# niclasborlin/dbat

Measured on AMD Instinct MI355X. Metric: LM iterations/sec, higher is better.
Workload: dtype f64

## Files before the change

### dbat_amd/csrc/dbat_core.hip

```cpp
#include <hip/hip_runtime.h>
#include <rocblas/rocblas.h>
#include <rocsolver/rocsolver.h>
#include <rccl/rccl.h>

#include <chrono>
#include <cmath>
#include <cstdio>
#include <cstdlib>
#include <memory>
#include <string>
#include <thread>
#include <type_traits>
#include <utility>
#include <atomic>
#include <vector>

#include "../../include/dbat_hip.h"
#include "chol_df.hpp"
#include "kernels.hpp"
#include "sig.hpp"
#include "heavy.hpp"
#include "plan.hpp"
#include "resect.hpp"
#include "robust.hpp"
// ... 492 lines not shown
            if (allreduce(allreduce_user, buf, count, (void *)stream) != 0) throw DeviceError{"all-reduce callback failed"};
        }
    }
    const double *gathered(const double *z_dev) {
        if (!multi()) return z_dev;
        if (!zgather.p) zgather.alloc((size_t)P.NZ);
        launch<k_mask_owned>(dim3((unsigned)cdiv(P.NZ, 256)), dim3(256), 0, P.NZ, z_mine.p, z_dev, zgather.p);
        do_allreduce(zgather.p, P.NZ);
        return zgather.p;
    }
    void read_scal(double *host, int n) {
        if (n <= 32) {
            HIPCHK(hipMemcpyAsync(hpin, scal.p, n * sizeof(double), hipMemcpyDeviceToHost, stream));
            sync();
            memcpy(host, hpin, n * sizeof(double));
            return;
        }
        HIPCHK(hipMemcpyAsync(host, scal.p, n * sizeof(double), hipMemcpyDeviceToHost, stream));
        sync();
    }
    void prep_cams(const double *zz, CamRec *into = nullptr) {
        if (!into) { into = cams.p; cams_at_lin = false; }
        launch<k_cam_prep>(dim3((unsigned)cdiv(P.nc, 64)), dim3(64), 0, d, zz, into);
    }
    void x_to_z(const double *x_host, double *z_dev) {
        HIPCHK(hipMemcpyAsync(z_dev, P.z0.data(), P.NZ * 8, hipMemcpyHostToDevice, stream));
        if (P.n) {
            HIPCHK(hipMemcpyAsync(xbuf.p, x_host, P.n * 8, hipMemcpyHostToDevice, stream));
            launch<k_scatter_x>(dim3((unsigned)cdiv(P.n, 256)), dim3(256), 0, P.n, x2z.p, xbuf.p, z_dev);
        }
    }
    void z_to_x(const double *z_dev, double *x_host) {
        if (!P.n) return;
        stage(4);
        z_dev = gathered(z_dev);
        launch<k_gather_x>(dim3((unsigned)cdiv(P.n, 256)), dim3(256), 0, P.n, x2z.p, z_dev, xbuf.p);
        HIPCHK(hipMemcpyAsync(x_host, xbuf.p, P.n * 8, hipMemcpyDeviceToHost, stream));
        sync();
    }

    DevBuf<double> trace_dev;
    int trace_cap = 0, trace_n = 0;
    std::vector<uint8_t> trace_have;
    void trace_begin() { trace_n = 0; trace_have.clear(); }
    void trace_put(int k, const double *z_dev) {
        if (!P.n || k < 0) return;
        if (k >= trace_cap) {
            const int cap = std::max(8, std::max(2 * trace_cap, k + 1));
            DevBuf<double> nb;
            nb.alloc((size_t)P.n * cap);
            if (trace_cap > 0) HIPCHK(hipMemcpyAsync(nb.p, trace_dev.p, (size_t)P.n * trace_cap * 8, hipMemcpyDeviceToDevice, stream));
            HIPCHK(hipStreamSynchronize(stream));
            std::swap(trace_dev.p, nb.p);
            trace_cap = cap;
        }
        stage(4);
        z_dev = gathered(z_dev);
        launch<k_gather_x>(dim3((unsigned)cdiv(P.n, 256)), dim3(256), 0, P.n, x2z.p, z_dev, trace_dev.p + (size_t)P.n * k);
        if ((int)trace_have.size() <= k) trace_have.resize((size_t)k + 1, 0);
        trace_have[k] = 1;
        trace_n = std::max(trace_n, k + 1);
    }
    void trace_truncate(int n) { trace_n = std::min(trace_n, std::max(n, 0)); }
    int trace_download(double *host, int cap_cols) {
        const int nt = std::min(trace_n, cap_cols);
        if (!P.n || nt <= 0) return std::max(nt, 0);
        HIPCHK(hipMemcpyAsync(host, trace_dev.p, (size_t)P.n * nt * 8, hipMemcpyDeviceToHost, stream));
        HIPCHK(hipStreamSynchronize(stream));
        for (int k = 0; k < nt; ++k)
            if (!trace_have[k]) std::fill(host + (size_t)P.n * k, host + (size_t)P.n * (k + 1), NAN);
        if ((size_t)P.n * trace_cap * 8 > ((size_t)256 << 20)) {
            DevBuf<double> old;
            std::swap(old.p, trace_dev.p);
            trace_cap = 0;
        }
        return nt;
    }

    double eval_f_step(const double *x, double alpha, const double *pdir, double *out) {
        stage(3);
        if ((int64_t)cdiv(P.NZ, 256) < P.nc) { axpby(1.0, x, alpha, pdir, out); return eval_f(out, nullptr, nullptr); }
        launch<k_axpby_cams>(dim3((unsigned)cdiv(P.NZ, 256)), dim3(256), 0, d, 1.0, x, alpha, pdir, out, cams_f.p);
        return eval_f(out, nullptr, nullptr, true);
    }
    double eval_f(const double *zz, double *r_w_out, double *r_unw_out, bool cams_ready = false) {
        stage(3);
        if (!cams_ready) prep_cams(zz, cams_f.p);
        mark(6);
        const bool res_tail = n_cm_chunks_all > 0 && n_cm_chunks_all <= 512 && !d.any_prior && !multi() && !r_w_out && !r_unw_out;
        with_value<2, 3, 4, 5>(P.model, [&](auto M) {
            with_value<false, true>(uv_pre, [&](auto PRE) {
                if (n_cm_chunks_all > 0)
                    launch<k_residual_cm<M, PRE>>(dim3((unsigned)n_cm_chunks_all), dim3(256), 0, d, zz, cams_f.p, cm_pt.p, cm_uv.p, pw ? cm_w.p : (const double *)nullptr,
                                                  cm_chunk_cam.p, cm_chunk_start.p, partial.p, res_tail ? gctr.p + 1 : (unsigned *)nullptr, scal.p, hpin, res_tail ? ++mb_seq : 0ull);
                mark(7);
                if (r_w_out || r_unw_out) launch<k_residual<M, PRE>>(dim3(grid_obs), dim3(256), 0, d, zz, cams_f.p, rpart.p, r_w_out, r_unw_out);
            });
        });
        if (!res_tail)
            launch<k_prior_sq>(dim3(grid_zs), dim3(1024), 0, d, zz, gpart.p, gctr.p + 1, (const double *)partial.p, n_cm_chunks_all,
                               scal.p, multi() ? (double *)nullptr : hpin, ++mb_seq);
        double s;
        if (multi()) { do_allreduce(scal.p, 1); read_scal(&s, 1); }
        else { mb_armed = true; sync(); s = hpin[0]; }
        ++n_res_evals;
        return 0.5 * s;
    }

    int det_ncx() const { return P.ncolmax <= 6 ? 6 : (P.ncolmax <= 14 ? 14 : 15); }
    bool deterministic_supported() const { return P.nranks == 1 && !P.shared_eo && P.ncolmax <= 15 && n_cm_chunks_all > 0; }
    void set_deterministic(bool on) {
        if (on && !deterministic_supported())
            throw UsageError{"deterministic mode: one rank, no shared EO blocks (camera stations), at most nine estimated IO columns per camera"};
        if (on && !det_u.p) {
            const int nc = P.nc;
            det_cam_part.alloc((size_t)std::max<int64_t>(n_cm_chunks_all, 1) * DET_CP);
            det_io_part.alloc((size_t)nc * DET_IOP);
            det_rr.alloc((size_t)nc + 1 + DET_PRIOR_PARTS);
            det_u.alloc((size_t)P.NS + 1);
            std::vector<int32_t> cr((size_t)2 * (2 * nc + 1), 0);
            for (int part = 0; part < 2; ++part) {
                const int64_t q0 = part == 0 ? 0 : n_cm_chunks, q1 = part == 0 ? n_cm_chunks : n_cm_chunks_all;
                int32_t *r = cr.data() + part * (2 * nc + 1);
                for (int c = 0; c < nc; ++c) { r[2 * c] = (int32_t)q1; r[2 * c + 1] = (int32_t)q1; }
                for (int64_t q = q0; q < q1; ++q) {
                    const int c = P.cm_chunk_cam[q];
                    if (r[2 * c] == (int32_t)q1) r[2 * c] = (int32_t)q;
                    r[2 * c + 1] = (int32_t)q + 1;
                }
                for (int c = 0; c < nc; ++c) if (r[2 * c] == (int32_t)q1) r[2 * c + 1] = (int32_t)q1;
            }
            det_cam_chunks.upload(cr);
        }
        deterministic = on;
        d.deterministic = on ? 1 : 0;
        d.det_cam_part = det_cam_part.p; d.det_io_part = det_io_part.p; d.det_rr = det_rr.p; d.det_u = det_u.p;
        d.det_cam_chunks = det_cam_chunks.p;
    }
    const double *det_z = nullptr;
    void det_camera_side() {
        const int nio = (int)P.nIOu;
        const int ncx = det_ncx();
        with_value<6, 14, 15>(ncx, [&](auto NCX) { launch<k_det_cam_reduce<NCX>>(dim3((unsigned)P.nc), dim3(256), 0, d, cams.p, S, g_c, g_red, diagU); });
        if (ncx > 6 && nio > 0) launch<k_det_io_reduce<15>>(dim3((unsigned)(nio * (nio + 1) / 2 + nio)), dim3(256), 0, d, cams.p, nio, S, g_c, g_red, diagU);
        if (d.any_prior) launch<k_det_prior_sq>(dim3(DET_PRIOR_PARTS), dim3(256), 0, d, det_z);
        launch<k_det_rows>(dim3((unsigned)cdiv(P.NS, 256)), dim3(256), 0, d, (const double *)diagU);
        if (ncx == 6) launch<k_det_round_cam<6>>(dim3((unsigned)P.nc), dim3(256), 0, d, cams.p, 0, S, g_red);
        else launch<k_det_round_cam<15>>(dim3((unsigned)P.nc + 1), dim3(256), 0, d, cams.p, nio, S, g_red);
    }

    void cam_normal(const double *zz, int64_t q0, int64_t nq, int ncx) {
        const double *w = pw ? cm_w.p : (const double *)nullptr;
        with_value<2, 3, 4, 5>(P.model, [&](auto M) { with_value<6, 14, 15>(ncx, [&](auto NCX) {
            if constexpr (NCX == 6)
                launch<k_cam_normal6<M>>(dim3((unsigned)nq), dim3(256), 0, d, zz, cams.p, cm_pt.p, cm_uv.p, w, cm_chunk_cam.p + q0, cm_chunk_start.p + q0, S, g_c, g_red, diagU);
            else
                launch<k_cam_normal<M, NCX>>(dim3((unsigned)nq), dim3(256), 0, d, zz, cams.p, cm_pt.p, cm_uv.p, w, cm_chunk_cam.p + q0, cm_chunk_start.p + q0, S, g_c, g_red, diagU);
        }); });
    }

    void build_enqueue(const double *zz, double lambda, int scale) {
        stage(0);
        const bool fused_first = !s_dense_dirty && P.NS >= P.nc;
        if (!fused_first) prep_cams(zz);
        else cams_at_lin = false;
        bool pivmm_set = false;
        if (s_dense_dirty) {
            HIPCHK(hipMemsetAsync(red.p, 0, red_count * sizeof(double), stream));
            s_dense_dirty = false;
        } else {
            launch<k_envelope_cams>(dim3((unsigned)P.NS), dim3(256), 0, d, zz, cams.p, S, ldS, (int)P.NS, env_tail0, col_bend.p, g_red, pivmm.p);
            pivmm_set = true;
        }
        if (!pivmm_set) HIPCHK(hipMemcpyAsync(pivmm.p, hpin + 48, 4 * sizeof(double), hipMemcpyHostToDevice, stream));
        int64_t npart = 0;
        const bool det_list = deterministic && route != TileRoute::sig;
        const int64_t nb_tiled = det_list ? 0 : P.nb_tiled;
        if (deterministic) {
            cam_normal(zz, 0, n_cm_chunks_all, det_ncx());
            det_z = zz;
            det_camera_side();
        }
        if (ntiles > 0 && nb_tiled > 0) {
            npart = ntiles;
            if (!deterministic && use_tile2 && tile_ncx <= 15 && n_cm_chunks > 0) cam_normal(zz, 0, n_cm_chunks, tile_ncx);
            mark(0);
            with_value<2, 3, 4, 5>(P.model, [&](auto M) {
                if (route == TileRoute::sig) {
                    with_value<6, 14>(tile_ncx, [&](auto NCX) { with_value<4, 5>(sig_rb, [&](auto RB) { with_value<false, true>(pw, [&](auto PW) {
                        launch<k_build_sig<M, RB, NCX, PW>>(dim3((unsigned)std::min<int64_t>(ntiles, n_cu)), dim3(64 * sig_waves(RB, NCX > 6)), sig_lds_bytes(RB, NCX > 6),
                                                            d, zz, cams.p, lambda, scale, S, g_red, Vinv.p, gp.p, jn2p.p, partial.p, pivmm.p, sg_chunk.p, sg_tile_chunk0.p,
                                                            sg_lc.p, sg_uv.p, PW ? sg_w.p : (const double *)nullptr, gctr.p + 5);
                    }); }); });
                } else if (route == TileRoute::tile3) {
                    launch<k_build_tile3<M, TILE3_PC, TILE3_NBUF>>(dim3((unsigned)ntiles), dim3(768), lds_tile3, d, zz, cams.p, lambda, scale, S, g_red, Vinv.p, gp.p,
                                                                   jn2p.p, partial.p, pivmm.p);
                } else {
                    with_value<14, 15>(tile_ncx, [&](auto NCX) {
                        launch<k_build_tile2<M, NCX, TILE2_PC, TILE2_NBUF>>(dim3((unsigned)ntiles), dim3(512), lds_tile2, d, zz, cams.p, lambda, scale, S, g_c, g_red,
                                                                            diagU, Vinv.p, gp.p, jn2p.p, partial.p, pivmm.p);
                    });
                }
            });
            mark(1);
        }
        const bool no_tiles = !(ntiles > 0 && nb_tiled > 0);
        if (no_tiles) mark(0);
        const int64_t nb_lists = use_heavy ? P.nb_tiled : nb;
        if (nb_lists > nb_tiled) {
            with_value<2, 3, 4, 5>(P.model, [&](auto M) { with_value<false, true>(P.with_io, [&](auto IO) {
                launch<k_build<M, IO>>(dim3((unsigned)(nb_lists - nb_tiled)), dim3(P.BT), lds_build, d, zz, cams.p, lambda, scale, S, g_c, g_red, diagU, Vinv.p, gp.p,
                                       jn2p.p, partial.p + npart, pivmm.p, (int)nb_tiled);
            }); });
            npart += nb_lists - nb_tiled;
        }
        if (use_heavy) {
            mark(10);
            if (!deterministic && n_cm_chunks_all > n_cm_chunks) cam_normal(zz, n_cm_chunks, n_cm_chunks_all - n_cm_chunks, tile_ncx);
            if (nb > P.nb_tiled) {
                with_value<2, 3, 4, 5>(P.model, [&](auto M) { with_value<6, 14, 15>(tile_ncx, [&](auto NCX) {
                    launch<k_heavy_z<M, NCX>>(dim3((unsigned)(nb - P.nb_tiled)), dim3(256), heavy_z_lds_bytes(NCX, P.hv_max_batch_slots, deterministic), d, hv, zz,
                                              cams.p, lambda, scale, hv_Z.p, Vinv.p, gp.p, jn2p.p, partial.p + npart, pivmm.p, (int)P.nb_tiled);
                }); });
                npart += nb - P.nb_tiled;
            }
            if (ngiant > 0) {
                with_value<2, 3, 4, 5>(P.model, [&](auto M) { with_value<6, 14, 15>(tile_ncx, [&](auto NCX) {
                    launch<k_heavy_z_giant<M, NCX>>(dim3((unsigned)ngiant), dim3(giant_threads), 0, d, hv, zz, cams.p, lambda, scale, hv_Z.p, Vinv.p, gp.p, jn2p.p,
                                                    partial.p + npart, pivmm.p);
                }); });
                npart += ngiant;
            }
            mark(11);
            launch<k_heavy_syrk>(dim3((unsigned)cdiv(hv.ntasks, 4)), dim3(256), 0, d, hv, (const double *)hv_Z.p, S, g_red);
            mark(12);
        }
        if (no_tiles) mark(1);
        if (ngiant > 0 && !use_heavy) {
            with_value<2, 3, 4, 5>(P.model, [&](auto M) { with_value<false, true>(P.with_io, [&](auto IO) {
                launch<k_build_giant<M, IO>>(dim3((unsigned)ngiant), dim3(giant_threads), 0, d, zz, cams.p, lambda, scale, S, g_c, g_red, diagU, Vinv.p, gp.p, jn2p.p,
                                             partial.p + npart, pivmm.p);
            }); });
            npart += ngiant;
        }
        if (deterministic && route == TileRoute::sig && !no_tiles) {
            HIPCHK(hipMemcpyAsync(hpin + 60, gctr.p + 7, sizeof(unsigned), hipMemcpyDeviceToHost, stream));
            det_timeout_pending = true;
        }
        if ((d.ablate & 32) && use_heavy && nb > P.nb_tiled) {
            unsigned long long h[16];
            HIPCHK(hipStreamSynchronize(stream));
            HIPCHK(hipMemcpyFromSymbol(h, HIP_SYMBOL(g_tile2_prof), sizeof(h)));
            static const char *nm[6] = {"evaluate", "V, g sums", "point blocks", "EO rows of Z", "IO rows of Z", "tail"};
            fprintf(stderr, "[heavy_z prof, us per batch (thread 0) avg over %d batches]", (int)(nb - P.nb_tiled));
            for (int i = 0; i < 6; ++i) fprintf(stderr, " %s=%.2f", nm[i], h[8 + i] * 0.01 / (double)std::max<int64_t>(nb - P.nb_tiled, 1));
            fprintf(stderr, "\n");
            for (int i = 8; i < 16; ++i) h[i] = 0;
            HIPCHK(hipMemcpyToSymbol(HIP_SYMBOL(g_tile2_prof), h, sizeof(h)));
        }
        if ((d.ablate & 32) && use_sig) {
            unsigned long long h[16];
            HIPCHK(hipStreamSynchronize(stream));
            HIPCHK(hipMemcpyFromSymbol(h, HIP_SYMBOL(g_tile2_prof), sizeof(h)));
            static const char *nm[8] = {"tile init", "chunk head", "pass 1", "pass 2 eval+write", "pass 2 mfma", "chunk flush", "wait for the tile", "tile flush"};
            fprintf(stderr, "[sig prof, us per tile (wave 0) avg over %d tiles]", (int)ntiles);
            for (int i = 0; i < 8; ++i) fprintf(stderr, " %s=%.2f", nm[i], h[i] * 0.01 / (double)std::max<int64_t>(ntiles, 1));
            fprintf(stderr, "\n");
            memset(h, 0, sizeof(h));
            HIPCHK(hipMemcpyToSymbol(HIP_SYMBOL(g_tile2_prof), h, sizeof(h)));
        } else if ((d.ablate & 32) && use_tile2) {
            unsigned long long h[16];
            HIPCHK(hipStreamSynchronize(stream));
            HIPCHK(hipMemcpyFromSymbol(h, HIP_SYMBOL(g_tile2_prof), sizeof(h)));
            static const char *nm[12] = {"stage(wait freed)", "P1", "pbarrier", "P2", "P3", "drain", "cons wait full", "cons zero+free", "tail/flush", "loop head", "cons product", "cons wait done"};
            fprintf(stderr, "[tile2 prof, us per tile avg over %d tiles]", (int)ntiles);
            for (int i = 0; i < 12; ++i) fprintf(stderr, " %s=%.2f", nm[i], h[i] * 0.01 / (double)std::max<int64_t>(ntiles, 1));
            fprintf(stderr, "\n");
            memset(h, 0, sizeof(h));
            HIPCHK(hipMemcpyToSymbol(HIP_SYMBOL(g_tile2_prof), h, sizeof(h)));
        }
        launch<k_build_tail>(dim3(grid_zs), dim3(1024), 0, d, zz, partial.p, npart, jn2p.p, gpart.p, gctr.p + 2, red_scal,
                zz != zlin.p ? zlin.p : (double *)nullptr);
    }
    bool pend_build = false;
    double pend_lambda = 0;
    int pend_scale = 0;
    void request_build(double lambda, int scale) {
        pend_build = true; pend_lambda = lambda; pend_scale = scale;
        lambda_lin = lambda; scale_lin = scale;
    }
    void ensure_build() {
        if (!pend_build) return;
        build(z.p, pend_lambda, pend_scale, true);
    }
    void settle_lin_point() {
        if (!pend_build) return;
        copy(zlin.p, z.p);
        cams_at_lin = false; s_valid = false; have_lin = true;
    }
    void allreduce_vectors() {
        if (!multi()) return;
        do_allreduce(g_c, 2 * P.NS + 8);
    }
    void trace_only_pass(const double *zz) {
        stage(0);
        prep_cams(zz);
        if (n_cm_chunks_all > 0) {
            with_value<2, 3, 4, 5>(P.model, [&](auto M) { with_value<6, 14, 15, MAXCOL>(tile_ncx, [&](auto NCX) {
                launch<k_trace_cm<M, NCX>>(dim3((unsigned)n_cm_chunks_all), dim3(256), 0, d, zz, cams.p, cm_pt.p, cm_uv.p, pw ? cm_w.p : (const double *)nullptr,
// ... 2376 lines not shown
```

### dbat_amd/csrc/kernels.hpp

```cpp
#pragma once
#include <hip/hip_runtime.h>

#include "model.hpp"

namespace dbat {

struct DevProblem {
    int nc, np, nIOrows, nK, nP, nIOu, ncolmax, BT;
    int64_t NS, NZ, nobs, nb;
    int64_t ldS;
    const int32_t *cam_ncol, *cam_col, *cam_iorow;
    const uint32_t *cam_eo_est;
    const int32_t *io_src;
    const double *io_fixed;
    const double *px;
    const double *cam_w;
    const uint8_t *z_est, *z_mine;
    const double *z_prw, *z_prv;
    const int32_t *o_cam, *o_pt;
    const double *o_uv;
    const double *o_uv_raw;
    int uv_pre;
    const double *o_w;
    const uint32_t *o_seg;
// ... 968 lines not shown
    const int k = (int)(o1 - o0);
    const int pt = d.o_pt[o0];
    double s[3] = {0, 0, 0};
    for (int i = t; i < k; i += BT) {
        const int64_t o = o0 + i;
        const CamRec &C = cams[d.o_cam[o]];
        const int ncol = WITH_IO ? C.ncol : 6;
        double r[2], E[2][NCX], B[2][3], tt[2] = {0, 0};
        eval_obs_cols<MODEL, WITH_IO>(d, C, z, o, pt, r, E, B);
#pragma unroll
        for (int a = 0; a < NCX; ++a)
            if (a < ncol) { const double dc = dz[C.col[a]]; tt[0] += E[0][a] * dc; tt[1] += E[1][a] * dc; }
        s[0] = fma2(s[0], B[0][0], tt[0], B[1][0], tt[1]);
        s[1] = fma2(s[1], B[0][1], tt[0], B[1][1], tt[1]);
        s[2] = fma2(s[2], B[0][2], tt[0], B[1][2], tt[1]);
    }
    block_sum<3>(s, sh);
    if (t == 0) {
        for (int q = 0; q < 3; ++q) s[q] += gp[3 * (int64_t)pt + q];
        double p0, p1, p2;
        point_block_solve_neg(Vinv + 6 * (int64_t)pt, s[0], s[1], s[2], p0, p1, p2);
        const int64_t zp = d.NS + 3 * (int64_t)pt;
        dps[0] = d.z_est[zp] ? p0 : 0.0; dps[1] = d.z_est[zp + 1] ? p1 : 0.0; dps[2] = d.z_est[zp + 2] ? p2 : 0.0;
        dz[zp] = dps[0]; dz[zp + 1] = dps[1]; dz[zp + 2] = dps[2];
    }
    __syncthreads();
    double acc[2] = {0, 0};
    for (int i = t; i < k; i += BT) {
        const int64_t o = o0 + i;
        const CamRec &C = cams[d.o_cam[o]];
        const int ncol = WITH_IO ? C.ncol : 6;
        double r[2], E[2][NCX], B[2][3], tt[2] = {0, 0};
        eval_obs_cols<MODEL, WITH_IO>(d, C, z, o, pt, r, E, B);
#pragma unroll
        for (int a = 0; a < NCX; ++a)
            if (a < ncol) { const double dc = dz[C.col[a]]; tt[0] += E[0][a] * dc; tt[1] += E[1][a] * dc; }
        const double j0 = tt[0] + B[0][0] * dps[0] + B[0][1] * dps[1] + B[0][2] * dps[2];
        const double j1 = tt[1] + B[1][0] * dps[0] + B[1][1] * dps[1] + B[1][2] * dps[2];
        acc[0] = fma2(acc[0], j0, j0, j1, j1);
    }
    block_sum<2>(acc, sh);
    if (t == 0) { partial[2 * blockIdx.x] = acc[0]; partial[2 * blockIdx.x + 1] = acc[1]; }
}

typedef double mfma_d4 __attribute__((ext_vector_type(4)));
constexpr int TILE_LD = 144;

__device__ __forceinline__ void lds_fence() {
    __builtin_amdgcn_s_waitcnt(0xc07f);
    asm volatile("" ::: "memory");
}

template <int MODEL, int NCX>
__global__ __launch_bounds__(256, 3) void k_cam_normal(DevProblem d, const double *__restrict__ z,
                                                       const CamRec *__restrict__ cams,
                                                       const int32_t *__restrict__ cm_pt, const double *__restrict__ cm_uv,
                                                       const double *__restrict__ cm_w,
                                                       const int32_t *__restrict__ chunk_cam,
                                                       const int64_t *__restrict__ chunk_start, double *__restrict__ S,
                                                       double *__restrict__ g_c, double *__restrict__ g_red,
                                                       double *__restrict__ diagU) {
    constexpr bool IO = NCX > 6;
    constexpr int GLD = 66;
    __shared__ double Gl[4 * 16 * GLD];
    const int t = threadIdx.x, lane = t & 63, w = t >> 6;
    const int cam = chunk_cam[blockIdx.x];
    const int64_t q0 = chunk_start[blockIdx.x], q1 = chunk_start[blockIdx.x + 1];
    const CamRec &C = cams[cam];
    const int ncol = IO ? min(C.ncol, NCX) : 6;
    double *Gw = Gl + w * 16 * GLD;
    for (int c = NCX + 1; c < 16; ++c) Gw[c * GLD + lane] = 0.0;
    mfma_d4 acc = {0, 0, 0, 0};
    {
        auto load_obs = [&](int64_t q, int &pt, double2 &uv, double2 &ww) {
            pt = 0; uv = double2{0, 0}; ww = double2{C.w[0], C.w[1]};
            if (q < q1) {
                pt = cm_pt[q];
                uv = reinterpret_cast<const double2 *>(cm_uv)[q];
                if (cm_w) ww = reinterpret_cast<const double2 *>(cm_w)[q];
            }
        };
        const int64_t qw = q0 + 64 * w + lane;
        int pt_a, pt_b;
        double2 uv_a, uv_b, w_a, w_b;
        load_obs(qw, pt_a, uv_a, w_a);
        load_obs(qw + 256, pt_b, uv_b, w_b);
        double Qn[3];
        { const int64_t zp = d.NS + 3 * (int64_t)pt_a; Qn[0] = z[zp]; Qn[1] = z[zp + 1]; Qn[2] = z[zp + 2]; }
        const int prow = lane & 31;
        const double *ga = Gw + (lane & 15) * GLD + (lane >> 4);
        for (int64_t base = q0 + 64 * w; base < q1; base += 256) {
            const int64_t q = base + lane;
            const double Q[3] = {Qn[0], Qn[1], Qn[2]};
            const double2 uv = uv_a, ww = w_a;
            pt_a = pt_b; uv_a = uv_b; w_a = w_b;
            { const int64_t zp = d.NS + 3 * (int64_t)pt_a; Qn[0] = z[zp]; Qn[1] = z[zp + 1]; Qn[2] = z[zp + 2]; }
            load_obs(q + 512, pt_b, uv_b, w_b);
            double r[2] = {0, 0}, E[2][NCX];
#pragma unroll
            for (int c = 0; c < NCX; ++c) { E[0][c] = 0.0; E[1][c] = 0.0; }
            if (q < q1) {
                double B[2][3];
                eval_obs_pre<MODEL, NCX>(d, C, Q, uv.x, uv.y, ww.x, ww.y, 7u, r, E, B);
            }
#pragma unroll
            for (int half = 0; half < 2; ++half) {
                if ((lane >> 5) == half) {
                    if (ncol == NCX) {
#pragma unroll
                        for (int c = 0; c < NCX; ++c) { Gw[c * GLD + prow] = E[0][c]; Gw[c * GLD + 32 + prow] = E[1][c]; }
                    } else {
#pragma unroll
                        for (int c = 0; c < NCX; ++c) {
                            const bool on = c < ncol;
                            Gw[c * GLD + prow] = on ? E[0][c] : 0.0;
                            Gw[c * GLD + 32 + prow] = on ? E[1][c] : 0.0;
                        }
                    }
                    Gw[NCX * GLD + prow] = r[0]; Gw[NCX * GLD + 32 + prow] = r[1];
                }
                lds_fence();
                if (base + 32 * half < q1) {
                    double av[16];
#pragma unroll
                    for (int kk = 0; kk < 16; ++kk) av[kk] = ga[4 * kk];
#pragma unroll
                    for (int kk = 0; kk < 16; ++kk) acc = __builtin_amdgcn_mfma_f64_16x16x4f64(av[kk], av[kk], acc, 0, 0, 0);
                }
                lds_fence();
            }
        }
    }
    double *Gs = Gl;
    __syncthreads();
#pragma unroll
    for (int e = 0; e < 4; ++e) Gs[w * 256 + ((lane >> 4) + 4 * e) * 16 + (lane & 15)] = acc[e];
    __syncthreads();
    const int i = t >> 4, j = t & 15;
    const double g = (Gs[t] + Gs[256 + t]) + (Gs[512 + t] + Gs[768 + t]);
    if (d.deterministic) { d.det_cam_part[(int64_t)blockIdx.x * DET_CP + t] = g; return; }
    if (i < ncol && g != 0.0) {
        const int64_t ri = C.col[i];
        if (j < ncol) {
            const int64_t rj = C.col[j];
            if (i > j) atomic_add_f64(S + (ri >= rj ? rj * d.ldS + ri : ri * d.ldS + rj), g);
            else if (i == j) { atomic_add_f64(S + ri * d.ldS + ri, g); atomic_add_f64(diagU + ri, g); }
        } else if (j == NCX) {
            atomic_add_f64(g_c + ri, g);
            atomic_add_f64(g_red + ri, g);
        }
    }
}

template <int MODEL>
__global__ __launch_bounds__(256) void k_cam_normal6(DevProblem d, const double *__restrict__ z,
                                                     const CamRec *__restrict__ cams,
                                                     const int32_t *__restrict__ cm_pt, const double *__restrict__ cm_uv,
                                                     const double *__restrict__ cm_w,
                                                     const int32_t *__restrict__ chunk_cam,
                                                     const int64_t *__restrict__ chunk_start, double *__restrict__ S,
                                                     double *__restrict__ g_c, double *__restrict__ g_red,
                                                     double *__restrict__ diagU) {
    __shared__ double Gs[4 * 28];
    __shared__ double Rd[4][14 * 65];
    const int t = threadIdx.x, lane = t & 63, w = t >> 6;
    const int cam = chunk_cam[blockIdx.x];
    const int64_t q0 = chunk_start[blockIdx.x], q1 = chunk_start[blockIdx.x + 1];
    const CamRec &C = cams[cam];
    double G[28];
#pragma unroll
    for (int i = 0; i < 28; ++i) G[i] = 0.0;
    const double2 *uvp = reinterpret_cast<const double2 *>(cm_uv), *wp = reinterpret_cast<const double2 *>(cm_w);
    for (int64_t qb = q0 + t; qb < q1; qb += 4 * 256) {
        int pt[4]; double2 uv[4], ww[4]; double Qv[4][3];
#pragma unroll
        for (int u = 0; u < 4; ++u) {
            const int64_t q = qb + 256 * u;
            const bool on = q < q1;
            pt[u] = on ? cm_pt[q] : -1;
            uv[u] = on ? uvp[q] : double2{0, 0};
            ww[u] = (on && cm_w) ? wp[q] : double2{C.w[0], C.w[1]};
        }
#pragma unroll
        for (int u = 0; u < 4; ++u) {
            const double *p = z + d.NS + 3 * (int64_t)(pt[u] < 0 ? 0 : pt[u]);
            Qv[u][0] = p[0]; Qv[u][1] = p[1]; Qv[u][2] = p[2];
        }
#pragma unroll
        for (int u = 0; u < 4; ++u) {
            if (pt[u] < 0) continue;
            const double d0 = Qv[u][0] - C.c[0], d1 = Qv[u][1] - C.c[1], d2 = Qv[u][2] - C.c[2];
            const double X0 = C.Mt[0] * d0 + C.Mt[1] * d1 + C.Mt[2] * d2;
            const double X1 = C.Mt[3] * d0 + C.Mt[4] * d1 + C.Mt[5] * d2;
            const double X2 = C.Mt[6] * d0 + C.Mt[7] * d1 + C.Mt[8] * d2;
            const double iz = recip(X2);
            const double ph0 = X0 * iz, ph1 = X1 * iz;
            const double nf = -C.f, sc = nf * iz, s0 = sc * ww[u].x, s1 = sc * ww[u].y;
            const double r0 = (nf * ph0 - uv[u].x) * ww[u].x, r1 = (nf * ph1 - uv[u].y) * ww[u].y;
            double y[3][3];
            angle_terms(C, d0, d1, d2, X0, X1, X2, y);
            double e0[6], e1[6];
#pragma unroll
            for (int k = 0; k < 3; ++k) {
                e0[k] = -s0 * (C.Mt[k] - ph0 * C.Mt[6 + k]);      e1[k] = -s1 * (C.Mt[3 + k] - ph1 * C.Mt[6 + k]);
                e0[3 + k] = s0 * (y[k][0] - ph0 * y[k][2]);       e1[3 + k] = s1 * (y[k][1] - ph1 * y[k][2]);
            }
            int n = 0;
#pragma unroll
            for (int i = 0; i < 6; ++i)
#pragma unroll
                for (int j = 0; j <= i; ++j, ++n) G[n] = __builtin_fma(e0[i], e0[j], __builtin_fma(e1[i], e1[j], G[n]));
#pragma unroll
            for (int i = 0; i < 6; ++i) G[21 + i] = __builtin_fma(e0[i], r0, __builtin_fma(e1[i], r1, G[21 + i]));
            G[27] = __builtin_fma(r0, r0, __builtin_fma(r1, r1, G[27]));
        }
    }
#pragma unroll
    for (int h = 0; h < 2; ++h) {
#pragma unroll
        for (int v = 0; v < 14; ++v)
            Rd[w][v * 65 + lane] = G[14 * h + v];
        lds_fence();
        __builtin_amdgcn_wave_barrier();
        const int v = lane & 15, q4 = lane >> 4;
        double sum = 0.0;
        if (v < 14) {
#pragma unroll
            for (int i = 0; i < 16; ++i) sum += Rd[w][v * 65 + 16 * q4 + i];
        }
        sum += __shfl_xor(sum, 16, 64);
        sum += __shfl_xor(sum, 32, 64);
        if (lane < 14) Gs[w * 28 + 14 * h + lane] = sum;
        lds_fence();
        __builtin_amdgcn_wave_barrier();
    }
    __syncthreads();
    if (d.deterministic) {
        if (t < 28) d.det_cam_part[(int64_t)blockIdx.x * DET_CP + t] = (Gs[t] + Gs[28 + t]) + (Gs[56 + t] + Gs[84 + t]);
        return;
    }
    if (t < 27) {
        double g = (Gs[t] + Gs[28 + t]) + (Gs[56 + t] + Gs[84 + t]);
        int i = t - 21, j = i;
        if (t < 21) {
            i = 0;
            while ((i + 1) * (i + 2) / 2 <= t) ++i;
            j = t - i * (i + 1) / 2;
        }
        if (!((C.eo_est >> i) & (C.eo_est >> j) & 1u)) g = 0.0;
        if (g != 0.0) {
            if (t < 21) {
                const int64_t ri = C.col[i], rj = C.col[j];
                if (i == j) { atomic_add_f64(S + ri * d.ldS + ri, g); atomic_add_f64(diagU + ri, g); }
                else atomic_add_f64(S + (ri >= rj ? rj * d.ldS + ri : ri * d.ldS + rj), g);
            } else {
                const int64_t ri = C.col[t - 21];
                atomic_add_f64(g_c + ri, g);
                atomic_add_f64(g_red + ri, g);
            }
        }
    }
}

template <int NCX>
__global__ __launch_bounds__(256) void k_det_cam_reduce(DevProblem d, const CamRec *__restrict__ cams, double *__restrict__ S,
                                                        double *__restrict__ g_c, double *__restrict__ g_red,
                                                        double *__restrict__ diagU) {
    const int cam = blockIdx.x, t = threadIdx.x;
    const CamRec &C = cams[cam];
    const int nel = NCX == 6 ? 28 : 256;
    double g = 0.0;
    if (t < nel) {
        for (int part = 0; part < 2; ++part) {
            const int q0 = d.det_cam_chunks[2 * cam + part * (2 * d.nc + 1)], q1 = d.det_cam_chunks[2 * cam + 1 + part * (2 * d.nc + 1)];
            for (int q = q0; q < q1; ++q) g += d.det_cam_part[(int64_t)q * DET_CP + t];
        }
    }
    if constexpr (NCX == 6) {
        if (t == 27) d.det_rr[cam] = g;
        if (t < 27) {
            int i = t - 21, j = i;
            if (t < 21) {
                i = 0;
                while ((i + 1) * (i + 2) / 2 <= t) ++i;
                j = t - i * (i + 1) / 2;
            }
            if (!((C.eo_est >> i) & (C.eo_est >> j) & 1u)) g = 0.0;
            if (t < 21) {
                const int64_t ri = C.col[i], rj = C.col[j];
                if (((C.eo_est >> i) & (C.eo_est >> j) & 1u)) {
                    S[(ri >= rj ? rj * d.ldS + ri : ri * d.ldS + rj)] = g;
                    if (i == j) diagU[ri] = g;
                }
            } else if ((C.eo_est >> i) & 1u) {
                const int64_t ri = C.col[i];
                g_c[ri] = g; g_red[ri] = g;
            }
        }
    } else {
        const int ncol = min(C.ncol, NCX);
        const int i = t >> 4, j = t & 15;
        if (i == NCX && j == NCX) d.det_rr[cam] = g;
        double *iop = d.det_io_part + (int64_t)cam * DET_IOP;
        if (i < ncol) {
            const int64_t ri = C.col[i];
            if (j < ncol && i >= j) {
                if (j >= 6) iop[(i - 6) * 9 + (j - 6)] = g;
                else {
                    const int64_t rj = C.col[j];
                    S[(ri >= rj ? rj * d.ldS + ri : ri * d.ldS + rj)] = g;
                    if (i == j) diagU[ri] = g;
                }
            } else if (j == NCX) {
                if (i >= 6) iop[81 + (i - 6)] = g;
                else { g_c[ri] = g; g_red[ri] = g; }
            }
        }
    }
}

template <int NCX>
__global__ __launch_bounds__(256) void k_det_io_reduce(DevProblem d, const CamRec *__restrict__ cams, int nio, double *__restrict__ S,
                                                       double *__restrict__ g_c, double *__restrict__ g_red,
                                                       double *__restrict__ diagU) {
    __shared__ double sh[256];
    const int npair = nio * (nio + 1) / 2, e = blockIdx.x, t = threadIdx.x;
    int p, q;
    if (e < npair) { p = 0; while ((p + 1) * (p + 2) / 2 <= e) ++p; q = e - p * (p + 1) / 2; }
    else { p = e - npair; q = -1; }
    const int64_t rp = 6 * (int64_t)d.nc + p, rq = 6 * (int64_t)d.nc + q;
    double s = 0.0;
    for (int c = t; c < d.nc; c += 256) {
        const CamRec &C = cams[c];
        const int ncol = min(C.ncol, NCX);
        int a = -1, b = -1;
        for (int k = 6; k < ncol; ++k) { if (C.col[k] == rp) a = k; if (C.col[k] == rq) b = k; }
        if (a < 0) continue;
        const double *iop = d.det_io_part + (int64_t)c * DET_IOP;
        if (q < 0) s += iop[81 + (a - 6)];
        else if (b >= 0) s += iop[(max(a, b) - 6) * 9 + (min(a, b) - 6)];
    }
    sh[t] = s;
    __syncthreads();
    for (int w = 128; w > 0; w >>= 1) {
        if (t < w) sh[t] += sh[t + w];
        __syncthreads();
    }
    if (t == 0) {
        if (q < 0) { g_c[rp] = sh[0]; g_red[rp] = sh[0]; }
        else { S[rq * d.ldS + rp] = sh[0]; if (p == q) diagU[rp] = sh[0]; }
    }
}

constexpr int DET_PRIOR_PARTS = 256;
__global__ __launch_bounds__(256) void k_det_prior_sq(DevProblem d, const double *__restrict__ z) {
    __shared__ double sh[256];
    const int t = threadIdx.x;
    const int64_t per = (d.NZ + DET_PRIOR_PARTS - 1) / DET_PRIOR_PARTS;
    const int64_t lo = per * blockIdx.x, hi = lo + per < d.NZ ? lo + per : d.NZ;
    double s = 0.0;
    for (int64_t i = lo + t; i < hi; i += 256) {
        const double pw = d.z_prw[i];
        if (pw > 0) { const double e = z[i] - d.z_prv[i]; s += pw * e * e; }
    }
    sh[t] = s;
    __syncthreads();
    for (int w = 128; w > 0; w >>= 1) {
        if (t < w) sh[t] += sh[t + w];
// ... 1510 lines not shown
```

### dbat_amd/csrc/sig.hpp

```cpp
#pragma once
#include <cstddef>
#include <type_traits>

#include "kernels.hpp"

namespace dbat {

constexpr int SIG_LDK = 18;
constexpr int SIG_PPR = 6;
constexpr int SIG_KMAXR = 13;
constexpr int SIG_NW = 8;
constexpr int SIG_CAMW = (int)(offsetof(CamRec, ncol) / 8) + 1;
constexpr int SIG_CAMW_IO = (int)((sizeof(CamRec) + 7) / 8);
constexpr int SIG_STILE = 8064;
#ifndef DBAT_SIG_IO_WAVES
#define DBAT_SIG_IO_WAVES 4
#endif
constexpr int SIG_IO_CAMS = DBAT_SIG_IO_WAVES == 8 ? 16 : 21;
__host__ __device__ constexpr int sig_stile(bool io) { return io && DBAT_SIG_IO_WAVES == 8 ? 6336 : SIG_STILE; }
__host__ __device__ constexpr int sig_cams(bool io) { return io ? SIG_IO_CAMS : 21; }

struct SigLds {
    int next_chunk, abort_;
    int flush_turn;
// ... 526 lines not shown
                if (ks + 1 < 5) load_ops(ks + 1, nxt);
                if (ks < ksteps) {
#pragma unroll
                    for (int r1 = 0; r1 < RB; ++r1)
                        if (r1 < rbk) {
#pragma unroll
                            for (int r2 = 0; r2 <= r1; ++r2)
                                acc[r1 * (r1 + 1) / 2 + r2] = __builtin_amdgcn_mfma_f64_16x16x4f64(
                                    cur[r1], cur[r2], acc[r1 * (r1 + 1) / 2 + r2], 0, 0, 0);
                        }
                }
            }
            lds_fence();
            __builtin_amdgcn_wave_barrier();
            lap(4);
        }
        if (d.deterministic) {
            volatile int *turn = &sy.flush_turn;
            int spins = 0;
            for (; *turn != ch_cur - ch0 && spins < (1 << 24); ++spins) __builtin_amdgcn_s_sleep(1);
            if (spins >= (1 << 24) && lane == 0) atomicAdd(det_timeouts, 1u);
        }
        {
            const int r6k = ry;
            int tcm[RB];
#pragma unroll
            for (int r2 = 0; r2 < RB; ++r2) tcm[r2] = sy.tmap[wave][min(16 * r2 + (lane & 15), 79)];
#pragma unroll
            for (int r1 = 0; r1 < RB; ++r1) {
                if (r1 >= rbk) break;
#pragma unroll
                for (int e = 0; e < 4; ++e) {
                    const int lr = 16 * r1 + (lane >> 4) + 4 * e;
                    const bool yrow = lr == r6k;
                    double *row = stile + (yrow ? STILE : sy.toff[wave][min(lr, 79)]);
                    if (!DBAT_ABLATE(d, 8)) {
#pragma unroll
                        for (int r2 = 0; r2 < r1; ++r2) {
                            const double v = acc[r1 * (r1 + 1) / 2 + r2][e];
                            atomic_add_f64(row + tcm[r2], yrow ? -v : v);
                        }
                        const double v = acc[r1 * (r1 + 1) / 2 + r1][e];
                        const int lcol = 16 * r1 + (lane & 15);
                        if (lcol <= lr && lcol < r6k && v != 0.0) atomic_add_f64(row + tcm[r1], yrow ? -v : v);
                    }
                }
            }
        }
        if (d.deterministic) {
            lds_fence();
            if (lane == 0) { volatile int *turn = &sy.flush_turn; *turn = ch_cur - ch0 + 1; }
        }
        __builtin_amdgcn_wave_barrier();
        lap(5);
    }
    lap(6);
    __syncthreads();
    lap(6);
    {
        constexpr int NCOLW = (128 + NW - 1) / NW;
        double v0[NCOLW], v1[NCOLW];
#pragma unroll
        for (int q = 0; q < NCOLW; ++q) {
            const int tc = wave + q * NW, tr = tc + lane;
            v0[q] = (tc < nrows && tr < nrows) ? stile[tr * (tr + 1) / 2 + tc] : 0.0;
            v1[q] = (tc < nrows && tr + 64 < nrows) ? stile[(tr + 64) * (tr + 65) / 2 + tc] : 0.0;
            if (d.deterministic && tc < nrows) {
                const double uc = sy.urow[tc];
                if (tr < nrows) v0[q] = det_round(v0[q], sy.urow[tr], uc);
                if (tr + 64 < nrows) v1[q] = det_round(v1[q], sy.urow[tr + 64], uc);
            }
        }
        if (!DBAT_ABLATE(d, 16)) {
#pragma unroll
            for (int q = 0; q < NCOLW; ++q) {
                const int tc = wave + q * NW, tr = tc + lane;
                if (tc < nrows) {
                    const int64_t gcol = sy.grow[tc] * d.ldS;
                    if (v0[q] != 0.0) atomic_add_f64(S + gcol + sy.grow[tr], -v0[q]);
                    if (v1[q] != 0.0) atomic_add_f64(S + gcol + sy.grow[tr + 64], -v1[q]);
                }
            }
        }
    }
    for (int i = t; i < nrows; i += NT) {
        const double v = d.deterministic ? det_round(vt[i], sy.urow[i], sy.uf) : vt[i];
        if (v != 0.0) atomic_add_f64(g_red + sy.grow[i], v);
    }
    double accr[1] = {rr};
    block_sum<1>(accr, sh);
    if (t == 0) partial[part_slot] = accr[0];
    pmin = pmin < 1e300 ? sqrt(pmin) : pmin; pmax = sqrt(pmax);
    for (int off = 32; off > 0; off >>= 1) {
        pmin = fmin(pmin, __shfl_down(pmin, off, 64));
        pmax = fmax(pmax, __shfl_down(pmax, off, 64));
    }
    if ((t & 63) == 0 && pmax > 0.0) {
        atomicMin(pivmm, (unsigned long long)__double_as_longlong(pmin));
        atomicMax(pivmm + 1, (unsigned long long)__double_as_longlong(pmax));
    }
    lap(7);
    if (prof)
        for (int i = 0; i < 8; ++i) if (tp[i]) atomicAdd(&g_tile2_prof[i], (unsigned long long)tp[i]);
}

template <int MODEL, int RB, int NCX, bool PW>
__global__ __launch_bounds__(64 * sig_waves(RB, (NCX > 6))) void k_build_sig(DevProblem d, const double *__restrict__ z,
                                                   const CamRec *__restrict__ cams, double lambda, int scale,
                                                   double *__restrict__ S, double *__restrict__ g_red,
                                                   double *__restrict__ Vinv, double *__restrict__ gp,
                                                   double *__restrict__ jn2p,
                                                   double *__restrict__ partial, unsigned long long *__restrict__ pivmm,
                                                   const int32_t *__restrict__ sg_chunk,
                                                   const int32_t *__restrict__ sg_tile_chunk0,
                                                   const uint8_t *__restrict__ sg_lc, const double *__restrict__ sg_uv,
                                                   const double *__restrict__ sg_w, unsigned *__restrict__ tile_ctr) {
    __shared__ unsigned s_ticket;
    __shared__ SigLds sy;
    __shared__ double sh[16];
    for (;;) {
        if (threadIdx.x == 0) s_ticket = __hip_atomic_fetch_add(tile_ctr, 1u, __ATOMIC_RELAXED, __HIP_MEMORY_SCOPE_AGENT);
        __syncthreads();
        const unsigned ti = s_ticket;
        if (ti >= (unsigned)d.ntiles) {
            if (threadIdx.x == 0 && ti == (unsigned)d.ntiles + gridDim.x - 1)
                __hip_atomic_store(tile_ctr, 0u, __ATOMIC_RELAXED, __HIP_MEMORY_SCOPE_AGENT);
            return;
        }
        const int tile = d.tile_order[ti];
        int ios = 0;
        if constexpr (NCX > 6) ios = d.tile_io_simple ? d.tile_io_simple[tile] : 0;
#ifdef DBAT_SIG_ONLY_IOS
        ios = DBAT_SIG_ONLY_IOS;
#endif
        if (NCX > 6 && ios == 1)
            build_sig_tile<MODEL, RB, NCX, (NCX > 6 ? 1 : 0), PW>(d, tile, (int)ti, z, cams, lambda, scale, S, g_red, Vinv, gp, jn2p, partial, pivmm, sg_chunk, sg_tile_chunk0, sg_lc, sg_uv, sg_w, tile_ctr + 2, sy, sh);
        else if (NCX > 6 && ios == 2)
            build_sig_tile<MODEL, RB, NCX, (NCX > 6 ? 2 : 0), PW>(d, tile, (int)ti, z, cams, lambda, scale, S, g_red, Vinv, gp, jn2p, partial, pivmm, sg_chunk, sg_tile_chunk0, sg_lc, sg_uv, sg_w, tile_ctr + 2, sy, sh);
        else
            build_sig_tile<MODEL, RB, NCX, 0, PW>(d, tile, (int)ti, z, cams, lambda, scale, S, g_red, Vinv, gp, jn2p, partial, pivmm, sg_chunk, sg_tile_chunk0, sg_lc, sg_uv, sg_w, tile_ctr + 2, sy, sh);
        __syncthreads();
    }
}

template <int MODEL, int NCX>
__global__ __launch_bounds__(256) void k_backsub_sig(DevProblem d, const double *__restrict__ z,
                                                     const CamRec *__restrict__ cams,
                                                     const double *__restrict__ Vinv, const double *__restrict__ gp,
                                                     double *__restrict__ dz, double *__restrict__ partial ,
                                                     const int32_t *__restrict__ sg_chunk, int nchunks,
                                                     const int32_t *__restrict__ sg_gcam,
                                                     const double *__restrict__ sg_uv, const double *__restrict__ sg_w) {
    constexpr int CW = (int)((sizeof(CamRec) + 7) / 8);
    __shared__ double sh[8];
    __shared__ double crec[4][SIG_KMAXR][CW];
    __shared__ double dcs[4][SIG_KMAXR][NCX];
    const int t = threadIdx.x, lane = t & 63;
    const int wv = t >> 6;
    const int ch = __builtin_amdgcn_readfirstlane(blockIdx.x * 4 + (t >> 6));
    double acc[2] = {0, 0};
    if (ch < nchunks) {
        const int32_t *cd = sg_chunk + 8 * (int64_t)ch;
        const int pt0 = cd[0], npts = cd[1], k = cd[2], gm = cd[4], gi0 = cd[5], uv0 = cd[6];
        const int mycam = lane < k ? sg_gcam[16 * (int64_t)ch + lane] : 0;
        for (int base = 0; base < k * CW; base += 64) {
            const int idx = base + lane, c = min(idx / CW, k - 1), f = idx - c * CW;
            const int cam = __builtin_amdgcn_ds_bpermute(4 * c, mycam);
            if (idx < k * CW) crec[wv][c][f] = reinterpret_cast<const double *>(cams + cam)[f];
        }
        __builtin_amdgcn_wave_barrier();
        for (int idx = lane; idx < k * NCX; idx += 64) {
            const int c = idx / NCX, a = idx - c * NCX;
            const CamRec &C = *reinterpret_cast<const CamRec *>(crec[wv][c]);
            const bool on = a < (NCX > 6 ? min(C.ncol, NCX) : 6) && (NCX > 6 || ((C.eo_est >> a) & 1u));
            dcs[wv][c][a] = on ? dz[C.col[a]] : 0.0;
        }
        __builtin_amdgcn_wave_barrier();
        const int G = npts > 32 ? 64 : (npts > 16 ? 32 : (npts > 8 ? 16 : 8));
        const int pi = lane & (G - 1), jh = lane / G, jstep = 64 / G;
        const bool act = pi < npts;
        const int pt = pt0 + (act ? pi : 0);
        const int64_t zp = d.NS + 3 * (int64_t)pt;
        const double Q[3] = {z[zp], z[zp + 1], z[zp + 2]};
        const unsigned est = (d.z_est[zp] ? 1u : 0u) | (d.z_est[zp + 1] ? 2u : 0u) | (d.z_est[zp + 2] ? 4u : 0u);
        const double2 *uvp = reinterpret_cast<const double2 *>(sg_uv), *wp = reinterpret_cast<const double2 *>(sg_w);
        const int64_t q0 = uv0 + gi0 + (act ? pi : 0);
        double sB[3] = {0, 0, 0}, V0[6] = {0, 0, 0, 0, 0, 0}, tt2 = 0;
        auto sweep = [&](auto per_obs_w) {
        for (int j = jh; j < k; j += jstep) {
            const CamRec &C = *reinterpret_cast<const CamRec *>(crec[wv][j]);
            double2 uv = {0, 0};
            if constexpr (NCX > 6) uv = uvp[q0 + (int64_t)j * gm];
            double w0, w1;
            if constexpr (decltype(per_obs_w)::value) { const double2 ww = wp[q0 + (int64_t)j * gm]; w0 = ww.x; w1 = ww.y; }
            else { w0 = C.w[0]; w1 = C.w[1]; }
            double B[2][3], t0 = 0, t1 = 0;
            if constexpr (NCX > 6) {
                obs_step_dot<MODEL, true>(C, Q, uv.x, uv.y, w0, w1, est, dcs[wv][j], t0, t1, B);
            } else {
                sig_step_dot6(C, Q, w0, w1, dcs[wv][j], t0, t1, B);
            }
#define DBAT_ACC2(acc, a, b, c, e) acc = __builtin_fma(a, b, __builtin_fma(c, e, acc))
            DBAT_ACC2(tt2, t0, t0, t1, t1);
            DBAT_ACC2(sB[0], B[0][0], t0, B[1][0], t1);
            DBAT_ACC2(sB[1], B[0][1], t0, B[1][1], t1);
            DBAT_ACC2(sB[2], B[0][2], t0, B[1][2], t1);
            DBAT_ACC2(V0[0], B[0][0], B[0][0], B[1][0], B[1][0]);
            DBAT_ACC2(V0[1], B[0][0], B[0][1], B[1][0], B[1][1]);
            DBAT_ACC2(V0[2], B[0][0], B[0][2], B[1][0], B[1][2]);
            DBAT_ACC2(V0[3], B[0][1], B[0][1], B[1][1], B[1][1]);
            DBAT_ACC2(V0[4], B[0][1], B[0][2], B[1][1], B[1][2]);
            DBAT_ACC2(V0[5], B[0][2], B[0][2], B[1][2], B[1][2]);
#undef DBAT_ACC2
        }
        };
        if (sg_w) sweep(std::true_type{}); else sweep(std::false_type{});
        for (int m = G; m < 64; m <<= 1) {
#pragma unroll
            for (int c = 0; c < 3; ++c) sB[c] += lane_get(sB[c], lane ^ m);
#pragma unroll
            for (int c = 0; c < 6; ++c) V0[c] += lane_get(V0[c], lane ^ m);
            tt2 += lane_get(tt2, lane ^ m);
        }
        {
            const double s0 = gp[3 * (int64_t)pt] + sB[0], s1 = gp[3 * (int64_t)pt + 1] + sB[1], s2 = gp[3 * (int64_t)pt + 2] + sB[2];
            double p0, p1, p2;
            point_block_solve_neg(Vinv + 6 * (int64_t)pt, s0, s1, s2, p0, p1, p2);
            const double d0 = (est & 1u) ? p0 : 0.0, d1 = (est & 2u) ? p1 : 0.0, d2 = (est & 4u) ? p2 : 0.0;
            if (act && lane == pi) {
                dz[zp] = d0; dz[zp + 1] = d1; dz[zp + 2] = d2;
                acc[0] = tt2 + 2.0 * (d0 * sB[0] + d1 * sB[1] + d2 * sB[2])
                       + d0 * (V0[0] * d0 + V0[1] * d1 + V0[2] * d2) + d1 * (V0[1] * d0 + V0[3] * d1 + V0[4] * d2)
                       + d2 * (V0[2] * d0 + V0[4] * d1 + V0[5] * d2);
            }
        }
    }
    block_sum<2>(acc, sh);
    if (t == 0) { partial[2 * blockIdx.x] = acc[0]; partial[2 * blockIdx.x + 1] = acc[1]; }
}

}
```

Before: 631.9.

## Software-pipeline camera-normal loads and prefetch camera records in signature backsub

The 6-column camera normal kernel now runs a fixed three-stage software pipeline (index/uv loads, point gathers, math) over four batches of two observations. The per-observation weight path is specialised at compile time, and a static_assert ties the chunk size to this schedule. The signature back-substitution kernel reads its chunk descriptor and camera ids through one lane-parallel load plus readlane. It stages only the needed CamRec fields and camera deltas in registers before writing them to LDS, and issues the point gradient and Vinv loads early so their latency overlaps. The aim is to hide global-memory latency, at the cost of more registers and less generality (fixed chunk size, hardcoded CamRec field offsets).

```diff
diff --git a/dbat_amd/csrc/dbat_core.hip b/dbat_amd/csrc/dbat_core.hip
--- a/dbat_amd/csrc/dbat_core.hip
+++ b/dbat_amd/csrc/dbat_core.hip
@@ -668,9 +668,12 @@
     void cam_normal(const double *zz, int64_t q0, int64_t nq, int ncx) {
         const double *w = pw ? cm_w.p : (const double *)nullptr;
         with_value<2, 3, 4, 5>(P.model, [&](auto M) { with_value<6, 14, 15>(ncx, [&](auto NCX) {
-            if constexpr (NCX == 6)
-                launch<k_cam_normal6<M>>(dim3((unsigned)nq), dim3(256), 0, d, zz, cams.p, cm_pt.p, cm_uv.p, w, cm_chunk_cam.p + q0, cm_chunk_start.p + q0, S, g_c, g_red, diagU);
-            else
+            if constexpr (NCX == 6) {
+                static_assert(Plan::CM_CHUNK == 256 * 2 * CAMN6_NB, "k_cam_normal6: a lane's observations of a chunk, two per batch");
+                with_value<false, true>(pw, [&](auto PW) {
+                    launch<k_cam_normal6<M, PW>>(dim3((unsigned)nq), dim3(256), 0, d, zz, cams.p, cm_pt.p, cm_uv.p, w, cm_chunk_cam.p + q0, cm_chunk_start.p + q0, S, g_c, g_red, diagU);
+                });
+            } else
                 launch<k_cam_normal<M, NCX>>(dim3((unsigned)nq), dim3(256), 0, d, zz, cams.p, cm_pt.p, cm_uv.p, w, cm_chunk_cam.p + q0, cm_chunk_start.p + q0, S, g_c, g_red, diagU);
         }); });
     }
diff --git a/dbat_amd/csrc/kernels.hpp b/dbat_amd/csrc/kernels.hpp
--- a/dbat_amd/csrc/kernels.hpp
+++ b/dbat_amd/csrc/kernels.hpp
@@ -1144,7 +1144,8 @@
     }
 }
 
-template <int MODEL>
+constexpr int CAMN6_NB = 4;
+template <int MODEL, bool PW>
 __global__ __launch_bounds__(256) void k_cam_normal6(DevProblem d, const double *__restrict__ z,
                                                      const CamRec *__restrict__ cams,
                                                      const int32_t *__restrict__ cm_pt, const double *__restrict__ cm_uv,
@@ -1163,32 +1164,37 @@
 #pragma unroll
     for (int i = 0; i < 28; ++i) G[i] = 0.0;
     const double2 *uvp = reinterpret_cast<const double2 *>(cm_uv), *wp = reinterpret_cast<const double2 *>(cm_w);
-    for (int64_t qb = q0 + t; qb < q1; qb += 4 * 256) {
-        int pt[4]; double2 uv[4], ww[4]; double Qv[4][3];
-#pragma unroll
-        for (int u = 0; u < 4; ++u) {
-            const int64_t q = qb + 256 * u;
+    int pt[CAMN6_NB][2]; double2 uv[CAMN6_NB][2], ww[CAMN6_NB][2]; double Qv[CAMN6_NB][2][3];
+    auto stage_a = [&](int b) {
+#pragma unroll
+        for (int u = 0; u < 2; ++u) {
+            const int64_t q = q0 + t + 256 * (2 * b + u);
             const bool on = q < q1;
-            pt[u] = on ? cm_pt[q] : -1;
-            uv[u] = on ? uvp[q] : double2{0, 0};
-            ww[u] = (on && cm_w) ? wp[q] : double2{C.w[0], C.w[1]};
-        }
-#pragma unroll
-        for (int u = 0; u < 4; ++u) {
-            const double *p = z + d.NS + 3 * (int64_t)(pt[u] < 0 ? 0 : pt[u]);
-            Qv[u][0] = p[0]; Qv[u][1] = p[1]; Qv[u][2] = p[2];
-        }
-#pragma unroll
-        for (int u = 0; u < 4; ++u) {
-            if (pt[u] < 0) continue;
-            const double d0 = Qv[u][0] - C.c[0], d1 = Qv[u][1] - C.c[1], d2 = Qv[u][2] - C.c[2];
+            pt[b][u] = on ? cm_pt[q] : -1;
+            uv[b][u] = on ? uvp[q] : double2{0, 0};
+            if constexpr (PW) ww[b][u] = on ? wp[q] : double2{0, 0};
+        }
+    };
+    auto stage_b = [&](int b) {
+#pragma unroll
+        for (int u = 0; u < 2; ++u) {
+            const double *p = z + d.NS + 3 * (int64_t)(pt[b][u] < 0 ? 0 : pt[b][u]);
+            Qv[b][u][0] = p[0]; Qv[b][u][1] = p[1]; Qv[b][u][2] = p[2];
+        }
+    };
+    auto stage_c = [&](int b) {
+#pragma unroll
+        for (int u = 0; u < 2; ++u) {
+            if (pt[b][u] < 0) continue;
+            const double w0 = PW ? ww[b][u].x : C.w[0], w1 = PW ? ww[b][u].y : C.w[1];
+            const double d0 = Qv[b][u][0] - C.c[0], d1 = Qv[b][u][1] - C.c[1], d2 = Qv[b][u][2] - C.c[2];
             const double X0 = C.Mt[0] * d0 + C.Mt[1] * d1 + C.Mt[2] * d2;
             const double X1 = C.Mt[3] * d0 + C.Mt[4] * d1 + C.Mt[5] * d2;
             const double X2 = C.Mt[6] * d0 + C.Mt[7] * d1 + C.Mt[8] * d2;
             const double iz = recip(X2);
             const double ph0 = X0 * iz, ph1 = X1 * iz;
-            const double nf = -C.f, sc = nf * iz, s0 = sc * ww[u].x, s1 = sc * ww[u].y;
-            const double r0 = (nf * ph0 - uv[u].x) * ww[u].x, r1 = (nf * ph1 - uv[u].y) * ww[u].y;
+            const double nf = -C.f, sc = nf * iz, s0 = sc * w0, s1 = sc * w1;
+            const double r0 = (nf * ph0 - uv[b][u].x) * w0, r1 = (nf * ph1 - uv[b][u].y) * w1;
             double y[3][3];
             angle_terms(C, d0, d1, d2, X0, X1, X2, y);
             double e0[6], e1[6];
@@ -1206,6 +1212,13 @@
             for (int i = 0; i < 6; ++i) G[21 + i] = __builtin_fma(e0[i], r0, __builtin_fma(e1[i], r1, G[21 + i]));
             G[27] = __builtin_fma(r0, r0, __builtin_fma(r1, r1, G[27]));
         }
+    };
+    stage_a(0); stage_a(1); stage_b(0);
+#pragma unroll
+    for (int b = 0; b < CAMN6_NB; ++b) {
+        if (b + 2 < CAMN6_NB) stage_a(b + 2);
+        if (b + 1 < CAMN6_NB) stage_b(b + 1);
+        stage_c(b);
     }
 #pragma unroll
     for (int h = 0; h < 2; ++h) {
diff --git a/dbat_amd/csrc/sig.hpp b/dbat_amd/csrc/sig.hpp
--- a/dbat_amd/csrc/sig.hpp
+++ b/dbat_amd/csrc/sig.hpp
@@ -702,37 +702,86 @@
                                                      const int32_t *__restrict__ sg_gcam,
                                                      const double *__restrict__ sg_uv, const double *__restrict__ sg_w) {
     constexpr int CW = (int)((sizeof(CamRec) + 7) / 8);
+    constexpr int CWS = NCX > 6 ? CW : (int)(offsetof(CamRec, ncol) / 8);
+    constexpr int CWL = NCX > 6 ? CW : 17, CWF = (int)(offsetof(CamRec, f) / 8) + 1, CWW = (int)(offsetof(CamRec, w) / 8);
+    static_assert(CWF == 15 && CWW == 30, "k_backsub_sig: the fields of CamRec that sig_step_dot6 reads");
+    constexpr int NREC = (SIG_KMAXR * CWL + 63) / 64;
+    constexpr int NDC = (SIG_KMAXR * 6 + 63) / 64;
+    constexpr bool GR_EARLY = NCX == 6;
     __shared__ double sh[8];
-    __shared__ double crec[4][SIG_KMAXR][CW];
+    __shared__ double crec[4][SIG_KMAXR][CWS];
     __shared__ double dcs[4][SIG_KMAXR][NCX];
     const int t = threadIdx.x, lane = t & 63;
     const int wv = t >> 6;
     const int ch = __builtin_amdgcn_readfirstlane(blockIdx.x * 4 + (t >> 6));
     double acc[2] = {0, 0};
     if (ch < nchunks) {
-        const int32_t *cd = sg_chunk + 8 * (int64_t)ch;
-        const int pt0 = cd[0], npts = cd[1], k = cd[2], gm = cd[4], gi0 = cd[5], uv0 = cd[6];
-        const int mycam = lane < k ? sg_gcam[16 * (int64_t)ch + lane] : 0;
-        for (int base = 0; base < k * CW; base += 64) {
-            const int idx = base + lane, c = min(idx / CW, k - 1), f = idx - c * CW;
-            const int cam = __builtin_amdgcn_ds_bpermute(4 * c, mycam);
-            if (idx < k * CW) crec[wv][c][f] = reinterpret_cast<const double *>(cams + cam)[f];
-        }
-        __builtin_amdgcn_wave_barrier();
-        for (int idx = lane; idx < k * NCX; idx += 64) {
-            const int c = idx / NCX, a = idx - c * NCX;
-            const CamRec &C = *reinterpret_cast<const CamRec *>(crec[wv][c]);
-            const bool on = a < (NCX > 6 ? min(C.ncol, NCX) : 6) && (NCX > 6 || ((C.eo_est >> a) & 1u));
-            dcs[wv][c][a] = on ? dz[C.col[a]] : 0.0;
-        }
-        __builtin_amdgcn_wave_barrier();
+        int dsc = 0;
+        if (lane < 8) dsc = sg_chunk[8 * (int64_t)ch + lane];
+        else if (lane >= 16 && lane < 32) dsc = sg_gcam[16 * (int64_t)ch + lane - 16];
+        const int pt0 = __builtin_amdgcn_readlane(dsc, 0), npts = __builtin_amdgcn_readlane(dsc, 1);
+        const int k = __builtin_amdgcn_readlane(dsc, 2), gm = __builtin_amdgcn_readlane(dsc, 4);
+        const int gi0 = __builtin_amdgcn_readlane(dsc, 5), uv0 = __builtin_amdgcn_readlane(dsc, 6);
         const int G = npts > 32 ? 64 : (npts > 16 ? 32 : (npts > 8 ? 16 : 8));
         const int pi = lane & (G - 1), jh = lane / G, jstep = 64 / G;
         const bool act = pi < npts;
         const int pt = pt0 + (act ? pi : 0);
         const int64_t zp = d.NS + 3 * (int64_t)pt;
+        double rec[NREC], dc[NDC];
+        unsigned eo[NDC];
+#pragma unroll
+        for (int s = 0; s < NREC; ++s) {
+            const int idx = 64 * s + lane, c = min(idx / CWL, k - 1), fl = idx - c * CWL;
+            const int f = (CWL == CWS || fl < CWF) ? fl : fl - CWF + CWW;
+            const int cam = __builtin_amdgcn_ds_bpermute(4 * (16 + c), dsc);
+            rec[s] = 0.0;
+            if (idx < k * CWL) rec[s] = reinterpret_cast<const double *>(cams + cam)[f];
+        }
+#pragma unroll
+        for (int s = 0; s < NDC; ++s) {
+            const int idx = 64 * s + lane, c = min(idx / 6, k - 1), a = idx - 6 * c;
+            const int cam = __builtin_amdgcn_ds_bpermute(4 * (16 + c), dsc);
+            dc[s] = 0.0; eo[s] = 0;
+            if (idx < 6 * k) {
+                dc[s] = dz[6 * (int64_t)cam + a];
+                if constexpr (NCX == 6) eo[s] = cams[cam].eo_est;
+            }
+        }
         const double Q[3] = {z[zp], z[zp + 1], z[zp + 2]};
-        const unsigned est = (d.z_est[zp] ? 1u : 0u) | (d.z_est[zp + 1] ? 2u : 0u) | (d.z_est[zp + 2] ? 4u : 0u);
+        int64_t zp1 = zp + 1, zp2 = zp + 2;
+        asm volatile("" : "+v"(zp1), "+v"(zp2));
+        const unsigned char ze0 = d.z_est[zp], ze1 = d.z_est[zp1], ze2 = d.z_est[zp2];
+        double g[3] = {0, 0, 0}, R[6] = {0, 0, 0, 0, 0, 0};
+        if constexpr (GR_EARLY) {
+#pragma unroll
+            for (int c = 0; c < 3; ++c) g[c] = gp[3 * (int64_t)pt + c];
+#pragma unroll
+            for (int c = 0; c < 6; ++c) R[c] = Vinv[6 * (int64_t)pt + c];
+        }
+        {
+            double *cr = &crec[wv][0][0];
+#pragma unroll
+            for (int s = 0; s < NREC; ++s) {
+                const int idx = 64 * s + lane, c = idx / CWL, fl = idx - c * CWL;
+                const int f = (CWL == CWS || fl < CWF) ? fl : fl - CWF + CWW;
+                if (idx < k * CWL) cr[c * CWS + f] = rec[s];
+            }
+#pragma unroll
+            for (int s = 0; s < NDC; ++s) {
+                const int idx = 64 * s + lane, c = idx / 6, a = idx - 6 * c;
+                if (idx < 6 * k) dcs[wv][c][a] = (NCX > 6 || ((eo[s] >> a) & 1u)) ? dc[s] : 0.0;
+            }
+            if constexpr (NCX > 6) {
+                __builtin_amdgcn_wave_barrier();
+                for (int idx = lane; idx < k * (NCX - 6); idx += 64) {
+                    const int c = idx / (NCX - 6), a = 6 + idx - c * (NCX - 6);
+                    const CamRec &C = *reinterpret_cast<const CamRec *>(crec[wv][c]);
+                    dcs[wv][c][a] = a < min(C.ncol, NCX) ? dz[C.col[a]] : 0.0;
+                }
+            }
+            __builtin_amdgcn_wave_barrier();
+        }
+        const unsigned est = (ze0 ? 1u : 0u) | (ze1 ? 2u : 0u) | (ze2 ? 4u : 0u);
         const double2 *uvp = reinterpret_cast<const double2 *>(sg_uv), *wp = reinterpret_cast<const double2 *>(sg_w);
         const int64_t q0 = uv0 + gi0 + (act ? pi : 0);
         double sB[3] = {0, 0, 0}, V0[6] = {0, 0, 0, 0, 0, 0}, tt2 = 0;
@@ -773,9 +822,15 @@
             tt2 += lane_get(tt2, lane ^ m);
         }
         {
-            const double s0 = gp[3 * (int64_t)pt] + sB[0], s1 = gp[3 * (int64_t)pt + 1] + sB[1], s2 = gp[3 * (int64_t)pt + 2] + sB[2];
+            if constexpr (!GR_EARLY) {
+#pragma unroll
+                for (int c = 0; c < 3; ++c) g[c] = gp[3 * (int64_t)pt + c];
+#pragma unroll
+                for (int c = 0; c < 6; ++c) R[c] = Vinv[6 * (int64_t)pt + c];
+            }
+            const double s0 = g[0] + sB[0], s1 = g[1] + sB[1], s2 = g[2] + sB[2];
             double p0, p1, p2;
-            point_block_solve_neg(Vinv + 6 * (int64_t)pt, s0, s1, s2, p0, p1, p2);
+            point_block_solve_neg(R, s0, s1, s2, p0, p1, p2);
             const double d0 = (est & 1u) ? p0 : 0.0, d1 = (est & 2u) ? p1 : 0.0, d2 = (est & 4u) ? p2 : 0.0;
             if (act && lane == pi) {
                 dz[zp] = d0; dz[zp + 1] = d1; dz[zp + 2] = d2;
```

Measured after the change: 641.1, median of 6. Within noise of the previous version (+1.5%).
